# open-mmlab/Amphion

Hardware: AMD Instinct MI355X
Metric: audio samples/sec (HiFi-GAN V1 22.05 kHz generator, mel->wav) (higher is better)
Workload: dtype f32 (split-f16 MFMA: 3 x v_mfma_f32_32x32x16_f16 per term, f32 accumulate)

## Files before the change

### amphion_amd/_lib.py

```python
from __future__ import annotations

import ctypes
import os
import weakref
from ctypes import POINTER, c_char_p, c_float, c_int, c_int32, c_int64, c_size_t, c_void_p

_HERE = os.path.dirname(os.path.abspath(__file__))
LIB_PATH = os.environ.get("AMP_LIB_PATH") or os.path.join(_HERE, "lib", "libamphion_hip.so")

AMP_MAX_STAGES = 8
AMP_MAX_KERNELS = 8
AMP_MAX_DILATIONS = 8

AMP_ARCH_HIFIGAN, AMP_ARCH_BIGVGAN, AMP_ARCH_HIFIGAN_VITS = 0, 1, 2
AMP_ACT_LRELU, AMP_ACT_SNAKE, AMP_ACT_SNAKEBETA = 0, 1, 2
AMP_PRECISION_F32, AMP_PRECISION_F16X3 = 0, 1
AMP_CONV_OPT_PAD_REFLECT, AMP_CONV_OPT_TANH = 1, 2
AMP_PAD_REPLICATE, AMP_PAD_ZEROS, AMP_PAD_REFLECT = 0, 1, 2
AMP_PW_BIAS, AMP_PW_BIAS_GELU, AMP_PW_SCALE_RES = 0, 1, 2
PRECISIONS = {"f32": AMP_PRECISION_F32, "fp32": AMP_PRECISION_F32, "f16x3": AMP_PRECISION_F16X3}


class AmpError(RuntimeError):

# ... 19 lines not shown
        ("snake_logscale", c_int32),
        ("gin_channels", c_int32),
    ]


class amp_mel_desc(ctypes.Structure):
    _fields_ = [
        ("struct_size", ctypes.c_uint32),
        ("n_fft", c_int32),
        ("win_size", c_int32),
        ("hop_size", c_int32),
        ("n_mel", c_int32),
        ("pad_mode", c_int32),
        ("mag_eps", c_float),
        ("log_clip", c_float),
        ("mel_bands_dev", c_void_p),
        ("range_dev", c_void_p),
        ("range_host", c_void_p),
        ("range_reset_dev", c_void_p),
        ("range_seq", c_int32),
    ]

    def __init__(self, *args, **kw):
        super().__init__(ctypes.sizeof(type(self)), *args, **kw)


class amp_dw_desc(ctypes.Structure):
    _fields_ = [
        ("residual_channels", c_int32),
        ("residual_layers", c_int32),
        ("dilation_cycle_length", c_int32),
        ("n_mel", c_int32),
        ("upsample0", c_int32),
        ("upsample1", c_int32),
        ("max_steps", c_int32),
    ]


_SIGNATURES = {
    "amp_version": (c_int, []),
    "amp_last_error": (c_char_p, []),
    "amp_device_count": (c_int, []),
    "amp_set_precision": (c_int, [c_int]),
    "amp_get_precision": (c_int, []),
    "amp_gen_create": (c_int, [POINTER(amp_gen_desc), POINTER(c_void_p)]),
    "amp_gen_set_weight": (c_int, [c_void_p, c_char_p, c_void_p, POINTER(c_int64), c_int]),
    "amp_gen_finalize": (c_int, [c_void_p]),
    "amp_gen_hop": (c_int, [c_void_p]),
    "amp_gen_workspace_bytes": (c_size_t, [c_void_p, c_int, c_int]),
    "amp_set_group_mb": (c_int, [c_int]),
    "amp_set_pair_strips": (c_int, [c_int]),
    "amp_set_strip_fit": (c_int, [c_int]),
    "amp_pair_strip_plan": (c_int, [c_int, c_int, c_int, c_int, POINTER(c_int), POINTER(c_int), POINTER(c_int), POINTER(c_int)]),
    "amp_range_check": (c_int, [c_void_p]),
    "amp_gen_range_check": (c_int, [c_void_p, c_void_p]),
    "amp_gen_forward": (c_int, [c_void_p, c_void_p, c_void_p, c_int, c_int, c_void_p, c_void_p, c_size_t, c_void_p]),
    "amp_gen_forward_ragged": (c_int, [c_void_p, c_void_p, c_void_p, c_void_p, c_int, c_int, c_void_p, c_void_p, c_size_t, c_void_p]),
    "amp_gen_set_profiling": (c_int, [c_void_p, c_int]),
    "amp_gen_last_timing_ms": (c_int, [c_void_p, c_int, POINTER(c_float)]),
    "amp_gen_timing_ms": (c_int, [c_void_p, c_int, c_int, POINTER(c_float)]),
    "amp_gen_kernel_name": (c_int, [c_void_p, c_int, c_int, c_char_p, c_size_t]),
    "amp_gen_destroy": (None, [c_void_p]),
    "amp_conv_create": (c_int, [c_int, c_int, c_int, c_int, c_int, c_int, c_int, c_void_p, c_void_p, POINTER(c_void_p)]),
    "amp_conv_out_len": (c_int, [c_void_p, c_int]),
    "amp_conv_forward": (c_int, [c_void_p, c_void_p, c_int, c_int, c_float, c_void_p, c_float, c_void_p, c_void_p]),
    "amp_conv_forward_strided": (c_int, [c_void_p, c_void_p, ctypes.c_longlong, c_int, c_int, c_float, c_void_p, c_float, c_void_p, c_void_p]),
    "amp_conv_forward_ragged": (c_int, [c_void_p, c_void_p, ctypes.c_longlong, c_int, c_int, c_void_p, c_float, c_void_p, c_float, c_void_p, c_void_p]),
    "amp_conv_forward_mrf": (c_int, [c_void_p, c_void_p, c_int, c_int, c_float, c_void_p, c_void_p, c_int, c_float, c_void_p]),
    "amp_apnet_polar": (c_int, [c_void_p, c_void_p, c_void_p, c_size_t, c_void_p, c_void_p, c_void_p, c_void_p]),
    "amp_istft_same": (c_int, [POINTER(amp_mel_desc), c_void_p, c_void_p, c_int, c_int, c_void_p, c_void_p, c_void_p, c_void_p, c_void_p]),
    "amp_istft_same_polar": (c_int, [POINTER(amp_mel_desc), c_void_p, ctypes.c_longlong, c_int, c_int, c_float, c_void_p, c_void_p, c_void_p,
                                     c_void_p, c_void_p]),
    "amp_pw_create": (c_int, [c_int, c_int, c_void_p, c_void_p, POINTER(c_void_p)]),
    "amp_pw_forward": (c_int, [c_void_p, c_void_p, ctypes.c_longlong, c_int, c_int, c_int, c_void_p, c_void_p, c_void_p, c_void_p]),
    "amp_pw_precision": (c_int, [c_void_p]),
    "amp_pw_destroy": (None, [c_void_p]),
    "amp_dw_create": (c_int, [POINTER(amp_dw_desc), POINTER(c_void_p)]),
    "amp_dw_set_weight": (c_int, [c_void_p, c_char_p, c_void_p, ctypes.c_longlong]),
    "amp_dw_finalize": (c_int, [c_void_p]),
    "amp_dw_precision": (c_int, [c_void_p]),
    "amp_dw_set_precision": (c_int, [c_void_p, c_int]),
    "amp_dw_workspace_bytes": (c_size_t, [c_void_p, c_int, c_int]),
    "amp_dw_condition": (c_int, [c_void_p, c_void_p, c_int, c_int, c_void_p, c_void_p, c_size_t, c_void_p]),
    "amp_dw_embed": (c_int, [c_void_p, c_void_p, c_int, c_void_p, c_void_p]),
    "amp_dw_input": (c_int, [c_void_p, c_void_p, c_int, c_int, c_void_p, c_void_p]),
    "amp_dw_layer": (c_int, [c_void_p, c_int, c_void_p, c_void_p, c_void_p, ctypes.c_longlong, c_void_p, c_void_p, c_void_p, c_int, c_int, c_void_p]),
    "amp_dw_tail": (c_int, [c_void_p, c_void_p, c_int, c_int, c_void_p, c_void_p]),
    "amp_dw_forward": (c_int, [c_void_p, c_void_p, c_int, c_void_p, c_int, c_void_p, c_int, c_int, c_void_p, c_void_p, c_size_t, c_void_p]),
    "amp_dw_sample_step": (c_int, [c_void_p, c_void_p, c_int, c_float, c_float, c_float, c_float, c_void_p, c_void_p, c_int, c_int, c_void_p,
                                   c_size_t, c_void_p]),
    "amp_dw_destroy": (None, [c_void_p]),
    "amp_fvq_create": (c_int, [c_int, c_int, c_int, c_int, c_int, POINTER(c_void_p), POINTER(c_void_p), POINTER(c_void_p), POINTER(c_void_p),
                               POINTER(c_void_p), POINTER(c_void_p)]),
    "amp_fvq_encode": (c_int, [c_void_p, c_void_p, c_int, c_int, c_int, c_void_p, c_void_p, c_void_p, c_void_p]),
    "amp_fvq_decode": (c_int, [c_void_p, c_void_p, c_int, c_int, c_int, c_void_p, c_void_p]),
    "amp_fvq_check": (c_int, [c_void_p, c_void_p]),
    "amp_fvq_encode_ex": (c_int, [c_void_p, c_void_p, ctypes.c_longlong, c_void_p, c_int, c_int, c_int, c_void_p, c_void_p, c_void_p, c_void_p,
                                  c_void_p]),
    "amp_fvq_decode_add": (c_int, [c_void_p, c_void_p, c_int, c_int, c_int, c_void_p, c_void_p, c_void_p]),
    "amp_semantic_prepare": (c_int, [c_void_p, c_void_p, c_void_p, c_int, c_int, c_int, c_int, c_void_p, c_void_p]),
    "amp_fvq_destroy": (None, [c_void_p]),
    "amp_codec_unit_create": (c_int, [c_int, c_int, c_void_p, c_void_p, c_void_p, c_void_p, c_void_p, c_void_p, POINTER(c_void_p)]),
    "amp_codec_unit_fused": (c_int, [c_void_p]),
    "amp_set_codec_unit_fusion": (c_int, [c_int]),
    "amp_codec_unit_workspace_bytes": (c_size_t, [c_void_p, c_int, c_int]),
    "amp_codec_unit_forward": (c_int, [c_void_p, c_void_p, c_int, c_int, c_void_p, c_void_p, c_size_t, c_void_p]),
# ... 248 lines not shown
```

### amphion_amd/csrc/amp_host.h

```cpp
#pragma once
#include <math.h>

#include <vector>

#include "amp_internal.h"

#define AMP_HIP(expr)                                                                  \
    do {                                                                               \
        hipError_t e__ = (expr);                                                       \
        if (e__ != hipSuccess) {                                                       \
            set_error("%s failed: %s (%s:%d)", #expr, hipGetErrorString(e__), __FILE__, __LINE__); \
            return AMP_ERR_HIP;                                                        \
        }                                                                              \
    } while (0)

#define AMP_RC(expr) do { int rc__ = (expr); if (rc__ != AMP_OK) return rc__; } while (0)

struct amp_conv {
    int transposed = 0, cin = 0, cout = 0, k = 0, stride = 1, dilation = 1, padding = 0;
    int M = 0, ntaps = 0, KT = 0, off0 = 0, dstep = 0, halo_left = 0, halo_right = 0, up = 1, up_pad = 0;
    int nchunks = 0;
    int precision = amp::PREC_F32;
    int pad_reflect = 0, tanh_out = 0;
    int out_pad = 0;
// ... 4 lines not shown
    void* wp_dev = nullptr;
    float* bias_dev = nullptr;
    ~amp_conv() {
        if (wp_dev) (void)hipFree(wp_dev);
        if (bias_dev) (void)hipFree(bias_dev);
    }
};

struct amp_pw {
    int cin = 0, cout = 0;
    int precision = amp::PREC_F16X3;
    int nsteps = 0;
    float inv_scale = 1.f;
    uint4* wp_dev = nullptr;
    float* bias_dev = nullptr;
    amp_conv* conv = nullptr;
    ~amp_pw() {
        if (wp_dev) (void)hipFree(wp_dev);
        if (bias_dev) (void)hipFree(bias_dev);
        delete conv;
    }
};

namespace amp {

int device_upload(const void* host, size_t bytes, void** out);

struct DeviceAllocs {
    std::vector<void*> owned;
    DeviceAllocs() = default;
    DeviceAllocs(const DeviceAllocs&) = delete;
    DeviceAllocs& operator=(const DeviceAllocs&) = delete;
    ~DeviceAllocs() {
        for (void* p : owned) (void)hipFree(p);
    }
    int upload(const void* host, size_t bytes, void** out) {
        if (int rc = device_upload(host, bytes, out); rc != AMP_OK) return rc;
        owned.push_back(*out);
        return AMP_OK;
    }
    template <class T, class P>
    int upload(const std::vector<T>& v, P** out) { return upload(v.data(), v.size() * sizeof(T), (void**)out); }
};

int default_precision();

constexpr int kConvBlkDefault = 3;
constexpr int kConvRgFastDefault = 1;
constexpr int kPingPongDefault = 1;
struct Config {
    int pair_strips = -1;
    int strip_fit = -1;
    int rb_fusion = 1;
    int ampb_fusion = 1;
    int conv_blk = kConvBlkDefault;
    size_t group_bytes = 0;
    int small_conv = 1;
    int conv_rg_fast = 1;
    int pingpong = 1;
    int narrow_blk = 1;
    int rb_streams = -1;
    Config();
};
Config& cfg();

struct RangeGuard {
    unsigned* dev = nullptr;
    unsigned* host = nullptr;
    hipEvent_t ev = nullptr;
    bool pending = false;
};
bool guard_init(RangeGuard& g);
void guard_free(RangeGuard& g);
int range_poll(RangeGuard* g, hipStream_t st);
int range_publish(RangeGuard* g, hipStream_t st);
int range_check_sync(RangeGuard* g, hipStream_t st, const char* who);
struct RangeFlagScope {
    explicit RangeFlagScope(unsigned* word);
    ~RangeFlagScope();
    RangeFlagScope(const RangeFlagScope&) = delete;
    RangeFlagScope& operator=(const RangeFlagScope&) = delete;
};

inline float pow2_weight_scale(float wmax) {
    int e2 = 0;
    if (wmax > 0.f) { (void)frexpf(wmax, &e2); if (ldexpf(1.f, e2 - 1) == wmax) e2 -= 1; }
    return wmax > 0.f ? ldexpf(1.f, 13 - e2) : 1.f;
}

template <class View>
std::vector<_Float16> pack_a_f16x3(int row_blocks, int k16, int taps, size_t pad_entries, float wscale, View view) {
    std::vector<_Float16> wp(((size_t)row_blocks * k16 * taps * 2 + pad_entries) * 64 * 8, (_Float16)0.f);
    for (int mb = 0; mb < row_blocks; ++mb)
        for (int c = 0; c < k16; ++c)
            for (int g = 0; g < taps; ++g)
                for (int lane = 0; lane < 64; ++lane)
                    for (int e = 0; e < 8; ++e) {
                        const float v = view(mb * 32 + (lane & 31), c * 16 + 8 * (lane >> 5) + e, g) * wscale;
                        const _Float16 hi = (_Float16)v;
                        const _Float16 lo = (_Float16)(v - (float)hi);
                        const size_t ent = (((size_t)mb * k16 + c) * taps + g) * 2;
                        wp[((ent + 0) * 64 + lane) * 8 + e] = hi;
                        wp[((ent + 1) * 64 + lane) * 8 + e] = lo;
                    }
    return wp;
}

template <class View>
int pack_matrix_f16x3(const char* who, int rows, int cols, int row_blocks, int k16, View W, std::vector<_Float16>* wp, float* inv_scale) {
    float wmax = 0.f;
    for (int m = 0; m < rows; ++m)
        for (int i = 0; i < cols; ++i) {
            const float w = fabsf(W(m, i));
            if (!(w < 1e30f)) { set_error("%s: non-finite weight", who); return AMP_ERR_INVALID; }
            wmax = fmaxf(wmax, w);
        }
    const float wscale = pow2_weight_scale(wmax);
    *inv_scale = 1.f / (16.f * wscale);
    *wp = pack_a_f16x3(row_blocks, k16, 1, 0, wscale, [&](int m, int i, int) { return (m < rows && i < cols) ? W(m, i) : 0.f; });
    return AMP_OK;
}

int conv_build(amp_conv* c, const float* w, const float* bias);
int conv_run(const amp_conv* c, const float* x, int B, int T, float slope_in, const float* res, float slope_out, float* y, int mode, float div,
             hipStream_t stream, long long xbs = 0, const int* lens = nullptr, int len_mul = 1, ConvArgs* plan_small = nullptr,
             int* plan_ni = nullptr);
int next_rev(const int* lens);

bool pair_supported(const amp_conv* c1, const amp_conv* c2);
int pair_run(const amp_conv* c1, const amp_conv* c2, const float* x, int B, int T, float slope, float* y, int mode, float div,
             hipStream_t stream, const int* lens = nullptr, int len_mul = 1);
bool pair_strip_plan(int B, int T, int k, bool ragged, int* form, int* strip_len, int* spi, int* steps);
bool pair_tile_args(const amp_conv* c1, const amp_conv* c2, const float* x, int B, int T, float slope, float* y, int mode, float div,
                    const int* lens, int len_mul, PairArgs* out);

bool rb_supported(const amp_conv* const* c1, const amp_conv* const* c2, int np, int B, int T);
int rb_split(const amp_conv* const* c1, int np, int B, int T);
int rb_run(const amp_conv* const* c1, const amp_conv* const* c2, int np, const float* x, int B, int T, float slope, float* y, int mode,
           float div, hipStream_t stream, const int* lens = nullptr, int len_mul = 1, int first = 0, int count = -1);

struct ActParams {
    float* a_dev = nullptr;
    float* invb_dev = nullptr;
    float* fu_dev = nullptr;
    float* fd_dev = nullptr;
    float* fu2_dev = nullptr;
};
int act_params_upload(const float* alpha_dev, const float* beta_dev, int C, int logscale, const float* filt_up_host,
                      const float* filt_down_host, float** out);
bool ampb_supported(const amp_conv* const* c1, const amp_conv* const* c2, int np, const ActParams* acts, size_t nacts, int B, int T);
int ampb_run(const amp_conv* const* c1, const amp_conv* const* c2, int np, const ActParams* acts, const float* x, int B, int T, float* y,
             int mode, float div, hipStream_t stream, const int* lens = nullptr, int len_mul = 1);

}
```

### amphion_amd/csrc/amp_internal.h

```cpp
#pragma once
#include <hip/hip_runtime.h>
#include <stdarg.h>
#include <stdint.h>
#include <stdio.h>

#include <atomic>
#include <mutex>
#include <string>
#include <vector>

#include "amphion_hip.h"

namespace amp {

constexpr int KC = 8;
constexpr int KC16 = 16;

enum { PREC_F32 = 0, PREC_F16X3 = 1 };

struct ConvArgs {
    const float* x;
    const void* wp;
    const float* bias;
    const float* res;
// ... 27 lines not shown
    float* wn_x;
    float* wn_out;
    int wn_first, wn_last;
};

struct PairArgs {
    const float* x;
    float* y;
    const void* wp1;
    const float* bias1;
    const void* wp2;
    const float* bias2;
    int B, C, T;
    int tiles_per_item;
    int strip_len;
    int strips_per_item;
    int wide;
    int fit;
    int rev;
    int dil;
    float slope;
    float sc1, isc1, sc2, isc2;
    int mode;
    float div;
    const int* lens;
    int len_mul;
    unsigned* range_flag;
};

struct ConvSmall3Args {
    ConvArgs a[3];
    int nx[3], ny[3];
};
hipError_t launch_conv_small3(const ConvSmall3Args& p, const int ni[3], hipStream_t stream);

struct Pair3Args {
    PairArgs a[3];
    int n[3];
};
hipError_t launch_pair3(const Pair3Args& p, hipStream_t stream);

constexpr int AMP_RB_MAX_PAIRS = 3;
struct RbArgs {
    const float* x;
    float* y;
    const void* wp1[AMP_RB_MAX_PAIRS];
    const float* bias1[AMP_RB_MAX_PAIRS];
    const void* wp2[AMP_RB_MAX_PAIRS];
    const float* bias2[AMP_RB_MAX_PAIRS];
    float sc1[AMP_RB_MAX_PAIRS], isc1[AMP_RB_MAX_PAIRS], sc2[AMP_RB_MAX_PAIRS], isc2[AMP_RB_MAX_PAIRS];
    int dil[AMP_RB_MAX_PAIRS];
    int np;
    int rh;
    int B, C, T;
    int tiles_per_item;
    int rev;
    float slope;
    int mode;
    float div;
    const int* lens;
    int len_mul;
    unsigned* range_flag;
};

constexpr int AMP_AMPB_MAX_STEPS = 6;
struct AmpbArgs {
    const float* x;
    float* y;
    const void* wp[AMP_AMPB_MAX_STEPS];
    const float* bias[AMP_AMPB_MAX_STEPS];
    float sc[AMP_AMPB_MAX_STEPS], isc[AMP_AMPB_MAX_STEPS];
    int dil[AMP_AMPB_MAX_STEPS];
    const float* act_a[AMP_AMPB_MAX_STEPS];
    const float* act_invb[AMP_AMPB_MAX_STEPS];
    const float* act_fu[AMP_AMPB_MAX_STEPS];
    const float* act_fd[AMP_AMPB_MAX_STEPS];
    int ns;
    int rh;
    int B, C, T;
    int tiles_per_item;
    int rev;
    int mode;
    float div;
    const int* lens;
    int len_mul;
    unsigned* range_flag;
};

constexpr int DW_TN = 64;
struct DwLayerArgs {
    const float* x;
    const float* cond;
    const float* dconst;
    long long dconst_bs;
    const float* skip_in;
    float* x_out;
    float* skip_out;
    const uint4* wp1;
    const uint4* wp2;
    const float* w1f;
    const float* w2f;
    const float* bias1;
    const float* bias2;
    int C, n_mel, L, d;
    int K16;
    int tiles_per_item;
// ... 211 lines not shown
```

### amphion_amd/csrc/conv_host.hip

```cpp
#include <string.h>

#include <memory>
#include <type_traits>
#include <vector>

#include "amp_host.h"

namespace amp {

template <int... K> struct Taps { static constexpr int list[] = {K...}; };
using ConvTaps = Taps<1, 2, 3, 5, 7, 11>;
using BlkTaps = Taps<2, 3, 7, 11>;
using SmallTaps = Taps<1, 3, 5, 7, 11>;
using PairTaps = Taps<3, 5, 7, 11>;
using RbTaps = Taps<3, 5, 7, 11>;
using AmpbTaps = Taps<3, 5, 7, 11>;

template <int... K, typename R, typename F>
static R with_taps(Taps<K...>, int k, R dflt, F&& f) {
    R r = dflt;
    (void)((k == K && (r = f(std::integral_constant<int, K>{}), true)) || ...);
    return r;
}

// ... 376 lines not shown
    }
    const int NT = pair_tile(c1->k, c1->cin, c1->dilation);
    if (NT <= 0) return false;
    a.tiles_per_item = (T + NT - 1) / NT;
    *out = a;
    return true;
}

static int rb_fusion_mode() { return cfg().rb_fusion; }
static int rb_form(int C, int k) {
    const int m = rb_fusion_mode();
    if (m == 0) return -1;
    if (m == 3) return (C == 32 || (C == 64 && k <= 5)) ? 0 : 1;
    if (m == 2) return 1;
    if (C == 32) return k >= 11 ? 1 : 0;
    if (C == 64) return k <= 5 ? 0 : 1;
    if (C == 128) return 1;
    return -1;
}
constexpr long long kRbMinWorkgroups = 256;

bool rb_supported(const amp_conv* const* c1, const amp_conv* const* c2, int np, int B, int T) {
    if (np < 1 || np > AMP_RB_MAX_PAIRS) return false;
    int max_dil = 1, rh = 0;
    for (int p = 0; p < np; ++p) {
        if (!c1[p] || !c2[p] || !pair_supported(c1[p], c2[p])) return false;
        if (c1[p]->cin != c1[0]->cin || c1[p]->k != c1[0]->k) return false;
        max_dil = c1[p]->dilation > max_dil ? c1[p]->dilation : max_dil;
        rh += (c1[p]->k - 1) / 2 * (c1[p]->dilation + 1);
    }
    const int form = rb_form(c1[0]->cin, c1[0]->k);
    if (form < 0) return false;
    const int W = rb_tile(c1[0]->k, c1[0]->cin, max_dil, form);
    if (W <= 0 || W - 2 * rh < W / 2) return false;
    const int NT = W - 2 * rh;
    if (rb_fusion_mode() == 1 && (long long)B * ((T + NT - 1) / NT) < kRbMinWorkgroups) return false;
    return true;
}

int rb_split(const amp_conv* const* c1, int np, int B, int T) {
    if (np != 3 || rb_fusion_mode() != 1) return 0;
    int max_dil = 1, rh = 0;
    for (int p = 0; p < np; ++p) {
        max_dil = c1[p]->dilation > max_dil ? c1[p]->dilation : max_dil;
        rh += (c1[p]->k - 1) / 2 * (c1[p]->dilation + 1);
    }
    const int W = rb_tile(c1[0]->k, c1[0]->cin, max_dil, rb_form(c1[0]->cin, c1[0]->k));
    const int NT = W - 2 * rh;
    if (W <= 0 || 5 * NT >= 4 * W) return 0;
    if ((long long)B * ((T + NT - 1) / NT) < 1024) return 0;
    return 2;
}

int rb_run(const amp_conv* const* c1, const amp_conv* const* c2, int np, const float* x, int B, int T, float slope, float* y, int mode,
           float div, hipStream_t stream, const int* lens, int len_mul, int first, int count) {
    if (x == y) { set_error("rb_run: x and y must not alias"); return AMP_ERR_INVALID; }
    if (slope > 1.f) { set_error("rb_run: leaky_relu slope %g > 1 is outside the fused kernels", (double)slope); return AMP_ERR_UNSUPPORTED; }
    RbArgs a{};
    a.x = x; a.y = y;
    a.np = count < 0 ? np - first : count;
    c1 += first;
    c2 += first;
    int max_dil = 1;
    for (int p = 0; p < a.np; ++p) {
        a.wp1[p] = c1[p]->wp_dev; a.bias1[p] = c1[p]->bias_dev; a.wp2[p] = c2[p]->wp_dev; a.bias2[p] = c2[p]->bias_dev;
        a.sc1[p] = 16.f * c1[p]->wscale; a.isc1[p] = 1.f / a.sc1[p];
        a.sc2[p] = 16.f * c2[p]->wscale; a.isc2[p] = 1.f / a.sc2[p];
        a.dil[p] = c1[p]->dilation;
        a.rh += (c1[p]->k - 1) / 2 * (c1[p]->dilation + 1);
        max_dil = c1[p]->dilation > max_dil ? c1[p]->dilation : max_dil;
    }
    for (int p = a.np; p < AMP_RB_MAX_PAIRS; ++p) {
        a.wp1[p] = a.wp1[0]; a.bias1[p] = a.bias1[0]; a.wp2[p] = a.wp2[0]; a.bias2[p] = a.bias2[0]; a.dil[p] = 1;
    }
    a.B = B; a.C = c1[0]->cin; a.T = T;
    const int form = rb_form(a.C, c1[0]->k);
    const int W = rb_tile(c1[0]->k, a.C, max_dil, form);
    const int NT = W - 2 * a.rh;
    a.tiles_per_item = (T + NT - 1) / NT;
    a.slope = slope; a.mode = mode; a.div = div;
    a.lens = lens; a.len_mul = len_mul;
    a.range_flag = range_flag_for_current_device();
    a.rev = next_rev(lens);
    AMP_HIP(launch_rb(c1[0]->k, a, form, stream));
    return AMP_OK;
}

static int ampb_fusion_mode() { return cfg().ampb_fusion; }
static int ampb_form(int C, int k) {
    const int m = ampb_fusion_mode();
    if (m == 0) return -1;
    if (m == 3) return C == 32 ? 0 : 1;
    if (m == 2) return 1;
    if (C == 32) return k >= 11 ? 1 : 0;
    if (C == 64) return k <= 3 ? 1 : -1;
    return -1;
}
constexpr long long kAmpbMinWorkgroups = 256;

static int ampb_halo(const amp_conv* const* c1, int np) {
    int rh = 0;
    for (int p = 0; p < np; ++p) rh += 10 + (c1[p]->k - 1) / 2 * (c1[p]->dilation + 1);
    return (rh + 3) & ~3;
}

bool ampb_supported(const amp_conv* const* c1, const amp_conv* const* c2, int np, const ActParams* acts, size_t nacts, int B, int T) {
    if (np < 1 || 2 * np > AMP_AMPB_MAX_STEPS || nacts != (size_t)(2 * np)) return false;
    for (size_t i = 0; i < nacts; ++i)
        if (!acts[i].fu2_dev) return false;
    if ((T & 3) != 0) return false;
    int max_dil = 1;
    for (int p = 0; p < np; ++p) {
        const amp_conv *a = c1[p], *b = c2[p];
        if (!a || !b || a->precision != PREC_F16X3 || b->precision != PREC_F16X3) return false;
        if (a->pad_reflect || b->pad_reflect || a->tanh_out || b->tanh_out || a->transposed || b->transposed) return false;
        if (a->cin != a->cout || b->cin != b->cout || a->cin != b->cin || a->cin != c1[0]->cin) return false;
        if (a->k != c1[0]->k || b->k != a->k || b->dilation != 1 || a->k != a->KT) return false;
        if (a->padding != (a->k - 1) / 2 * a->dilation || b->padding != (b->k - 1) / 2) return false;
        if (!a->bias_dev || !b->bias_dev) return false;
        max_dil = a->dilation > max_dil ? a->dilation : max_dil;
    }
    const int form = ampb_form(c1[0]->cin, c1[0]->k);
    if (form < 0) return false;
    const int W = ampb_tile(c1[0]->k, c1[0]->cin, max_dil, form);
    const int rh = ampb_halo(c1, np);
    if (W <= 0 || W - 2 * rh < W / 2) return false;
    const int NT = W - 2 * rh;
    if (ampb_fusion_mode() == 1 && (long long)B * ((T + NT - 1) / NT) < kAmpbMinWorkgroups) return false;
    return true;
}
// ... 261 lines not shown
```

### amphion_amd/csrc/rb_f16x3.hip

```cpp
#include "f16x3_device.h"

#ifndef AMP_KT
#error "compile with -DAMP_KT=<taps>"
#endif

namespace amp {


template <int KT, int WM, int WN, int NI, int RING = 0, int RB_G = 32>
__global__ __launch_bounds__(64 * WM * WN, 2) void rb_f16x3_kernel(const RbArgs a) {
    static_assert(RING == 0 || RING < KT, "a ring shorter than one chunk");
    constexpr int NTHR = 64 * WM * WN;
    constexpr int W = 32 * NI * WN;
    constexpr int WL = W + 2 * RB_G;
    constexpr int H2 = (KT - 1) / 2;
    constexpr int NCH = 2 * WM;
    constexpr int CHS = 4 * WL;
    constexpr int C = 32 * WM;
    static_assert(NI % 2 == 0, "B fragments are read in halves");
    extern __shared__ __attribute__((aligned(16))) uint4 smem4[];

    const int tid = threadIdx.x;
    const int lane = tid & 63;
    const int wave = __builtin_amdgcn_readfirstlane(tid >> 6);
    const int wm = wave / WN, wn = wave % WN;
    const int hi = lane >> 5, l31 = lane & 31;
    const int nbx = gridDim.x;
    int bx = tile_order(blockIdx.x, nbx, a.lens != nullptr, a.rev);
    const int item = bx / a.tiles_per_item;
    const int tile = bx - item * a.tiles_per_item;
    const int T = a.T;
    const int RH = a.rh;
    const int NT = W - 2 * RH;
    const int O0 = tile * NT;
    int Tv = T;
    if (a.lens) { const int l = a.lens[item] * a.len_mul; Tv = l < Tv ? l : Tv; }
    if (O0 >= Tv) return;
    const int q0 = O0 - RH;

    for (int i = tid; i < NCH * 4 * 2 * RB_G; i += NTHR) {
        const int row = i / (2 * RB_G), g = i - row * (2 * RB_G);
        smem4[row * WL + (g < RB_G ? g : W + g)] = make_uint4(0u, 0u, 0u, 0u);
    }

    const int colw = wn * (32 * NI) + l31;
    int qcl[NI];
    bool qok[NI];
#pragma unroll
    for (int t = 0; t < NI; ++t) {
        const int q = q0 + colw + 32 * t;
        qok[t] = (q >= 0) && (q < Tv);
        qcl[t] = q < 0 ? 0 : (q < T ? q : T - 1);
    }
    const float* xr = a.x + (size_t)item * C * T + (size_t)(32 * wm + 16 * hi) * T;
    f32x16 rv[NI];
#pragma unroll
    for (int t = 0; t < NI; ++t)
#pragma unroll
        for (int r = 0; r < 16; ++r) rv[t][r] = xr[(size_t)r * T + qcl[t]];

    constexpr size_t MBS = (size_t)NCH * (KT * 128);
    constexpr int NA = RING > 0 ? RING : KT;
    Frag a_h[NA], a_l[NA];
    const int wlane = (lane & 32) | (16 * ((lane >> 2) & 1) + 4 * ((lane >> 3) & 3) + (lane & 3));
    {
        const uint4* w0 = static_cast<const uint4*>(a.wp1[0]) + (size_t)wm * MBS + wlane;
#pragma unroll
        for (int g = 0; g < NA; ++g) {
            a_h[g].u = w0[g * 128];
            a_l[g].u = w0[g * 128 + 64];
        }
    }
    AMP_PIN_VMEM();

    float range_max = 0.f;
    const float kpos = 16.f, kneg = 16.f * a.slope;
    auto stage_x = [&]() __attribute__((always_inline)) {
#pragma unroll
        for (int t = 0; t < NI; ++t) {
            const int col = RB_G + colw + 32 * t;
            const bool ok = qok[t];
            const int o4 = (2 * wm + hi) * CHS + col;
#pragma unroll
            for (int o = 0; o < 2; ++o) {
                struct { uint2 u; } fh0, fl0, fh1, fl1;
                stage4_f16(ok ? rv[t][8 * o + 0] : 0.f, ok ? rv[t][8 * o + 1] : 0.f, ok ? rv[t][8 * o + 2] : 0.f,
                           ok ? rv[t][8 * o + 3] : 0.f, kpos, kneg, range_max, fh0.u, fl0.u);
                stage4_f16(ok ? rv[t][8 * o + 4] : 0.f, ok ? rv[t][8 * o + 5] : 0.f, ok ? rv[t][8 * o + 6] : 0.f,
                           ok ? rv[t][8 * o + 7] : 0.f, kpos, kneg, range_max, fh1.u, fl1.u);
                smem4[o4 + o * WL] = make_uint4(fh0.u.x, fh0.u.y, fh1.u.x, fh1.u.y);
                smem4[o4 + o * WL + 2 * WL] = make_uint4(fl0.u.x, fl0.u.y, fl1.u.x, fl1.u.y);
            }
        }
    };

    f32x16 acc[NI];
    auto conv = [&](const void* wp, const float* bias, float sc, int d, const void* wp_next) __attribute__((always_inline)) {
#pragma unroll
        for (int r = 0; r < 16; ++r) {
            const float bv = bias[32 * wm + 16 * hi + r] * sc;
#pragma unroll
            for (int t = 0; t < NI; ++t) acc[t][r] = bv;
        }
        const uint4* wa = static_cast<const uint4*>(wp) + (size_t)wm * MBS + wlane;
        const uint4* wn0 = static_cast<const uint4*>(wp_next) + (size_t)wm * MBS + wlane;
        const int rd = hi * WL + RB_G + colw - H2 * d;
#pragma unroll 1
        for (int c = 0; c < NCH; ++c) {
            const uint4* wcur = wa + (size_t)c * (KT * 128);
            const uint4* wan = (c + 1) < NCH ? wa + (size_t)(c + 1) * (KT * 128) : wn0;
            const uint4* base = smem4 + c * CHS + rd;
#pragma unroll
            for (int g = 0; g < KT; ++g) {
                const int v = RING > 0 ? g % NA : g;
                const uint4* bg = base + g * d;
                constexpr int NB = NI / 2;
#pragma unroll
                for (int th = 0; th < 2; ++th) {
                    Frag bh[NB], bl[NB];
#pragma unroll
                    for (int t = 0; t < NB; ++t) {
                        bh[t].u = bg[32 * (th * NB + t)];
                        bl[t].u = bg[2 * WL + 32 * (th * NB + t)];
                    }
                    mfma3<NB>(acc + th * NB, a_h[v], a_l[v], bh, bl);
                }
                {
                    const bool same = RING > 0 && g + RING < KT;
                    const uint4* src = same ? wcur + (size_t)(g + RING) * 128 : wan + (size_t)v * 128;
                    a_h[v].u = src[0];
                    a_l[v].u = src[64];
                }
                AMP_PIN_VMEM();
            }
        }
    };

    stage_x();
    __syncthreads();

    const int np = a.np;
#pragma unroll 1
    for (int p = 0; p < AMP_RB_MAX_PAIRS; ++p) {
        if (p < np) {
            const bool last = (p + 1 == np);
            conv(a.wp1[p], a.bias1[p], a.sc1[p], a.dil[p], a.wp2[p]);
            __syncthreads();
            {
                const float i1 = a.isc1[p];
                const float slope = a.slope;
#pragma unroll
                for (int t = 0; t < NI; ++t) {
                    const int o4 = (2 * wm + hi) * CHS + RB_G + colw + 32 * t;
#pragma unroll
                    for (int o = 0; o < 2; ++o) {
                        struct { uint2 u; } fh0, fl0, fh1, fl1;
                        seam4_f16(acc[t][8 * o + 0], acc[t][8 * o + 1], acc[t][8 * o + 2], acc[t][8 * o + 3], i1, slope, qok[t], range_max, fh0.u, fl0.u);
                        seam4_f16(acc[t][8 * o + 4], acc[t][8 * o + 5], acc[t][8 * o + 6], acc[t][8 * o + 7], i1, slope, qok[t], range_max, fh1.u, fl1.u);
                        smem4[o4 + o * WL] = make_uint4(fh0.u.x, fh0.u.y, fh1.u.x, fh1.u.y);
                        smem4[o4 + o * WL + 2 * WL] = make_uint4(fl0.u.x, fl0.u.y, fl1.u.x, fl1.u.y);
                    }
                }
            }
            __syncthreads();
            conv(a.wp2[p], a.bias2[p], a.sc2[p], 1, last ? a.wp2[p] : a.wp1[p + 1 < AMP_RB_MAX_PAIRS ? p + 1 : p]);
            {
                const float i2 = a.isc2[p];
#pragma unroll
                for (int t = 0; t < NI; ++t)
#pragma unroll
                    for (int r = 0; r < 16; ++r) rv[t][r] = __builtin_fmaf(acc[t][r], i2, rv[t][r]);
            }
            if (!last) {
                __syncthreads();
                stage_x();
                __syncthreads();
            }
        }
    }

    {
        const int mode = a.mode;
        float* yr = a.y + (size_t)item * C * T + (size_t)(32 * wm + 16 * hi) * T;
        if (mode != 0) {
#pragma unroll
            for (int t = 0; t < NI; ++t)
#pragma unroll
                for (int r = 0; r < 16; ++r) acc[t][r] = yr[(size_t)r * T + qcl[t]];
#pragma unroll
            for (int t = 0; t < NI; ++t) rv[t] += acc[t];
            if (mode == 2) {
#pragma unroll
                for (int t = 0; t < NI; ++t)
#pragma unroll
                    for (int r = 0; r < 16; ++r) rv[t][r] = rv[t][r] / a.div;
            }
        }
#pragma unroll
        for (int t = 0; t < NI; ++t) {
            const int col = colw + 32 * t;
// ... 53 lines not shown
```

### amphion_amd/csrc/runtime.hip

```cpp
#include <stdarg.h>
#include <stdio.h>
#include <stdlib.h>
#include <string.h>

#include <mutex>
#include <string>

#include "amp_host.h"

namespace amp {

static thread_local char g_err[512] = "";

void set_error(const char* fmt, ...) {
    va_list ap;
    va_start(ap, fmt);
    vsnprintf(g_err, sizeof(g_err), fmt, ap);
    va_end(ap);
}

static RangeGuard g_guard[64];
__thread std::string* tl_kernel_log = nullptr;
__thread char tl_last_kernel[160] = "";
__thread int tl_conv_transposed = 0;
// ... 64 lines not shown

int range_poll(RangeGuard* g, hipStream_t st) {
    if (!g || !g->dev || !g->pending || stream_is_capturing(st)) return AMP_OK;
    if (hipEventQuery(g->ev) != hipSuccess) return AMP_OK;
    g->pending = false;
    if (*g->host == 0) return AMP_OK;
    *g->host = 0;
    AMP_HIP(hipMemsetAsync(g->dev, 0, sizeof(unsigned), st));
    set_error("%s", kRangeMsg);
    return AMP_ERR_RANGE;
}

int range_publish(RangeGuard* g, hipStream_t st) {
    if (!g || !g->dev || stream_is_capturing(st)) return AMP_OK;
    AMP_HIP(hipMemcpyAsync(g->host, g->dev, sizeof(unsigned), hipMemcpyDeviceToHost, st));
    AMP_HIP(hipEventRecord(g->ev, st));
    g->pending = true;
    return AMP_OK;
}

int range_check_sync(RangeGuard* g, hipStream_t st, const char* who) {
    if (!g || !g->dev) return AMP_OK;
    if (stream_is_capturing(st)) { set_error("%s: the stream is capturing", who); return AMP_ERR_STATE; }
    AMP_HIP(hipMemcpyAsync(g->host, g->dev, sizeof(unsigned), hipMemcpyDeviceToHost, st));
    AMP_HIP(hipStreamSynchronize(st));
    g->pending = false;
    const unsigned v = *g->host;
    *g->host = 0;
    if (v == 0) return AMP_OK;
    AMP_HIP(hipMemsetAsync(g->dev, 0, sizeof(unsigned), st));
    set_error("%s", kRangeMsg);
    return AMP_ERR_RANGE;
}

static int g_precision = -1;
int default_precision() {
    if (g_precision < 0) {
        const char* e = getenv("AMP_PRECISION");
        g_precision = (e && (!strcmp(e, "f32") || !strcmp(e, "fp32"))) ? PREC_F32 : PREC_F16X3;
    }
    return g_precision;
}

Config::Config() {
    auto num = [](const char* name, int lo, int hi, int dflt) {
        const char* e = getenv(name);
        if (!e || !*e) return dflt;
        const int v = atoi(e);
        return (v < lo || v > hi) ? dflt : v;
    };
    rb_fusion = num("AMP_RB_FUSION", 0, 3, 1);
    ampb_fusion = num("AMP_AMPB_FUSION", 0, 3, 1);
    rb_streams = num("AMP_RB_STREAMS", -1, 1, -1);
    static const char* const kRemoved[][2] = {
        {"AMP_GROUP_MB", "amp_set_group_mb(megabytes)"}, {"AMP_PAIR_STRIP", "amp_set_pair_strips(mode)"}, {"AMP_CONV_BLK", "amp_set_conv_blk(mode)"},
        {"AMP_FUSE_PAIRS", "nothing (the fused pairs are the only form)"}, {"AMP_RB_SUM_FRAMES", "nothing"},
        {"AMP_RB_HORIZONTAL", "amp_set_resblock_streams(mode)"}, {"AMP_RB_HORIZONTAL_FRAMES", "amp_set_resblock_streams(mode)"}};
    for (const auto& r : kRemoved) {
        const char* e = getenv(r[0]);
        if (e && *e) fprintf(stderr, "libamphion_hip: the environment variable %s=%s is no longer read (removed in ABI 142); use %s\n", r[0], e, r[1]);
    }
}
Config& cfg() { static Config c; return c; }

int device_upload(const void* host, size_t bytes, void** out) {
    void* p = nullptr;
    AMP_HIP(hipMalloc(&p, bytes));
    const hipError_t e = hipMemcpy(p, host, bytes, hipMemcpyHostToDevice);
    if (e != hipSuccess) {
        (void)hipFree(p);
        set_error("hipMemcpy of %zu bytes to the device failed: %s", bytes, hipGetErrorString(e));
        return AMP_ERR_HIP;
    }
    *out = p;
    return AMP_OK;
}

}

using namespace amp;

extern "C" {

int amp_version(void) { return 158; }
const char* amp_last_error(void) { return g_err; }

int amp_set_precision(int precision) {
    if (precision != AMP_PRECISION_F32 && precision != AMP_PRECISION_F16X3) {
        set_error("amp_set_precision: unknown precision %d", precision);
        return AMP_ERR_INVALID;
    }
    g_precision = precision;
    return AMP_OK;
}

int amp_get_precision(void) { return default_precision(); }

int amp_device_count(void) {
    int n = 0;
    if (hipGetDeviceCount(&n) != hipSuccess) return 0;
    return n;
}

int amp_set_pair_strips(int on) {
    if (on < -1 || on > 0) { set_error("amp_set_pair_strips: %d (-1 the policy, 0 the per-tile kernel everywhere; the four-wave strips of mode 1 left in ABI 142)", on); return AMP_ERR_INVALID; }
    cfg().pair_strips = on;
    return AMP_OK;
}

int amp_set_strip_fit(int mode) {
    if (mode < -1 || mode > 1) { set_error("amp_set_strip_fit: %d (-1 the plan, 0 never: shifted strips, 1 every strip launch)", mode); return AMP_ERR_INVALID; }
    cfg().strip_fit = mode;
    return AMP_OK;
}

int amp_pair_strip_plan(int B, int T, int k, int ragged, int* form, int* strip_len, int* strips_per_item, int* steps) {
    if (B < 1 || T < 1 || !form || !strip_len || !strips_per_item || !steps) { set_error("amp_pair_strip_plan: B=%d T=%d or a null result pointer", B, T); return AMP_ERR_INVALID; }
    if (!pair_strip_plan(B, T, k, ragged != 0, form, strip_len, strips_per_item, steps)) { set_error("amp_pair_strip_plan: no strip kernel for k=%d", k); return AMP_ERR_UNSUPPORTED; }
    return AMP_OK;
}

int amp_set_group_mb(int megabytes) {
    if (megabytes < 0) { set_error("amp_set_group_mb: %d", megabytes); return AMP_ERR_INVALID; }
    cfg().group_bytes = (size_t)megabytes << 20;
    return AMP_OK;
}

int amp_set_resblock_streams(int mode) {
    if (mode < -1 || mode > 1) { set_error("amp_set_resblock_streams: mode=%d", mode); return AMP_ERR_INVALID; }
    cfg().rb_streams = mode;
    return AMP_OK;
}

int amp_set_small_conv(int on) {
    cfg().small_conv = on ? 1 : 0;
    return AMP_OK;
}

int amp_set_pingpong(int on) {
    cfg().pingpong = on < 0 ? kPingPongDefault : (on ? 1 : 0);
    return AMP_OK;
}

int amp_set_conv_rg_fast(int on) {
    cfg().conv_rg_fast = on < 0 ? kConvRgFastDefault : (on ? 1 : 0);
    return AMP_OK;
}

int amp_set_conv_blk_narrow(int on) {
    if (on < -1 || on > 2) { set_error("amp_set_conv_blk_narrow: %d (0 off, 1 policy: 128-row convs with k >= 7, 2 every 128-row conv, -1 default)", on); return AMP_ERR_INVALID; }
    cfg().narrow_blk = on < 0 ? 1 : on;
    return AMP_OK;
}

int amp_set_conv_blk(int mode) {
    if (mode < -1 || mode > 3) { set_error("amp_set_conv_blk: mode %d (0 off, 1 | 2 chunks per staging round, 3 = 2 + k = 7 / 11, -1 default)", mode); return AMP_ERR_INVALID; }
    cfg().conv_blk = mode < 0 ? kConvBlkDefault : mode;
    return AMP_OK;
}

int amp_set_resblock_fusion(int mode) {
    if (mode < -1 || mode > 3) { set_error("amp_set_resblock_fusion: mode=%d", mode); return AMP_ERR_INVALID; }
    cfg().rb_fusion = mode < 0 ? 1 : mode;
    return AMP_OK;
}

int amp_set_ampblock_fusion(int mode) {
    if (mode < -1 || mode > 3) { set_error("amp_set_ampblock_fusion: mode=%d", mode); return AMP_ERR_INVALID; }
    cfg().ampb_fusion = mode < 0 ? 1 : mode;
    return AMP_OK;
}

int amp_range_check(void* stream_) {
    return range_check_sync(guard_for_current_device(), (hipStream_t)stream_, "amp_range_check");
// ... 4 lines not shown
```

### include/amphion_hip.h

```cpp
#ifndef AMPHION_HIP_H
#define AMPHION_HIP_H

#include <stddef.h>
#include <stdint.h>

#ifdef __cplusplus
extern "C" {
#endif

typedef enum amp_status {
    AMP_OK = 0,
    AMP_ERR_INVALID = -1,
    AMP_ERR_MISSING_WEIGHT = -2,
    AMP_ERR_HIP = -3,
    AMP_ERR_UNSUPPORTED = -4,
    AMP_ERR_STATE = -5,
    AMP_ERR_RANGE = -6
} amp_status;

typedef enum amp_arch {
    AMP_ARCH_HIFIGAN = 0,
    AMP_ARCH_BIGVGAN = 1,
    AMP_ARCH_HIFIGAN_VITS = 2
} amp_arch;
// ... 109 lines not shown
int amp_dwconv_layer_norm_c_causal(const float* x_dev, const float* dw_weight_dev, const float* dw_bias_dev, int K, int dilation,
                                   const float* gamma_dev, const float* beta_dev, const int* lens_dev, int B, int C, int T, float eps,
                                   int gelu, float* y_dev, void* stream);
int amp_dds_seam(const float* y_dev, const float* x_dev, const float* gamma2_dev, const float* beta2_dev, float eps2,
                 const float* dw_weight_dev, const float* dw_bias_dev, int K, int dilation, const float* gamma1_dev, const float* beta1_dev,
                 float eps1, const int* lens_dev, int B, int C, int T, float* x_out_dev, float* z_out_dev, void* stream);
int amp_add_channel_bias(float* x_dev, const float* cb_dev, int B, int C, int T, void* stream);
int amp_rel_attention(const float* q_dev, const float* k_dev, const float* v_dev, const float* emb_k_dev,
                      const float* emb_v_dev, const int* lens_dev, int B, int H, int dk, int T, int window, float* out_dev,
                      void* stream);
int amp_rel_attention_strided(const float* q_dev, const float* k_dev, const float* v_dev, long long qkv_batch_stride,
                              const float* emb_k_dev, const float* emb_v_dev, const int* lens_dev, int B, int H, int dk, int T,
                              int window, float* out_dev, void* stream);
int amp_set_rel_attention_tiled(int on);
int amp_dwconv(const float* x_dev, const float* w_dev, const float* bias_dev, const int* lens_dev, int B, int C, int T, int K,
               int dilation, float* y_dev, void* stream);
int amp_spline_flow(const float* z_dev, const float* h_dev, const int* lens_dev, int B, int T, int num_bins,
                    int filter_channels, float tail_bound, int inverse, int flip_in, int flip_out, float* z_out_dev,
                    void* stream);
int amp_spline_flow_proj(const float* z_dev, const float* hc_dev, const float* proj_w_dev, const float* proj_b_dev, const int* lens_dev,
                         int B, int C, int T, int num_bins, int filter_channels, float tail_bound, int inverse, int flip_in, int flip_out,
                         float* z_out_dev, void* stream);
int amp_affine_reverse(const float* x_dev, const float* m_dev, const float* logs_dev, const int* lens_dev, int B, int C, int T,
                       float* y_dev, void* stream);
int amp_embed_tokens(const long long* tokens_dev, const float* weight_dev, const int* lens_dev, int B, int T, int hidden,
                     int n_vocab, float scale, float* y_dev, void* stream);
int amp_embed_sum_c(const long long* codes_dev, int N, const float* const* tables, const int* rows, int D, const float* init_dev, int B, int T,
                    float* y_dev, unsigned* flag_dev, void* stream);
int amp_embed_sum_check(unsigned* flag_dev, void* stream);
int amp_durations(const float* logw_dev, const int* lens_dev, int B, int T, float length_scale, float* w_ceil_dev, int* cum_dev,
                  int* ylen_dev, void* stream);
int amp_expand_path(const float* src_dev, const int* cum_dev, const int* xlens_dev, const int* ylens_dev, int B, int D, int Tx,
                    int Ty, float* out_dev, float* attn_dev, void* stream);
int amp_expand_path_strided(const float* src_dev, long long src_batch_stride, const int* cum_dev, const int* xlens_dev,
                            const int* ylens_dev, int B, int D, int Tx, int Ty, float* out_dev, float* attn_dev, void* stream);
int amp_gauss_sample(const float* m_dev, const float* logs_dev, const float* noise_dev, size_t n, float noise_scale,
                     float* out_dev, void* stream);

int amp_snake(const float* x_dev, int B, int C, int T, const float* alpha_dev, const float* beta_dev, int logscale,
              float* y_dev, void* stream);

int amp_wav_to_pcm16(const float* wav_dev, int B, int L, long long wav_stride, const int* lens_dev, int16_t* pcm_dev,
                     long long pcm_stride, void* stream);

typedef enum amp_conv_option { AMP_CONV_OPT_PAD_REFLECT = 1, AMP_CONV_OPT_TANH = 2 } amp_conv_option;
int amp_conv_set_option(amp_conv* c, int option, int value);

int amp_pair_forward(const amp_conv* c1, const amp_conv* c2, const float* x_dev, int B, int T, float slope,
                     float* y_dev, void* stream);

int amp_resblock_forward(const amp_conv* const* c1, const amp_conv* const* c2, int n_pairs, const float* x_dev, int B, int T,
                         float slope, float* y_dev, void* stream);
int amp_set_resblock_fusion(int mode);
int amp_set_resblock_streams(int mode);
int amp_gen_prepare_streams(amp_gen* g);

int amp_ampblock_forward(const amp_conv* const* c1, const amp_conv* const* c2, int n_pairs, const float* alpha_dev,
                         const float* beta_dev, int logscale, const float* filt_up_host, const float* filt_down_host,
                         const float* x_dev, int B, int T, float* y_dev, int mode, float div, void* stream);
int amp_set_ampblock_fusion(int mode);

void amp_conv_destroy(amp_conv* c);

int amp_set_small_conv(int on);

int amp_set_conv_blk(int mode);
int amp_set_conv_blk_narrow(int on);

int amp_set_conv_rg_fast(int on);

int amp_set_pingpong(int on);


int amp_conv_create_gated(int hidden, int k, int dilation, int padding, const float* weight_host, const float* bias_host,
                          amp_conv** out);

int amp_wn_forward(const amp_conv* const* in_layers, const amp_conv* const* res_skip_layers, int n_layers, float* x_dev,
                   const float* cond_dev, long long cond_batch_stride, const int32_t* lens_dev, int B, int T,
                   float* acts_ws_dev, float* out_dev, void* stream);


int amp_wn_gate(const float* a_dev, const float* cond_dev, long long cond_batch_stride, float* out_dev, int B, int H,
                int T, void* stream);
int amp_wn_accumulate(float* x_dev, float* out_dev, const float* rs_dev, const int32_t* lens_dev, int B, int H, int T,
                      int first, int last, void* stream);
int amp_sequence_mask(float* x_dev, const int32_t* lens_dev, int B, int C, int T, void* stream);
int amp_coupling_apply(float* x_dev, const float* m_dev, const int32_t* lens_dev, int B, int half_channels, int T,
                       int reverse, void* stream);
int amp_flip_channels(const float* x_dev, float* y_dev, int B, int C, int T, void* stream);
int amp_posterior_sample(const float* stats_dev, const float* eps_dev, const int32_t* lens_dev, float* z_dev, int B,
                         int C, int T, void* stream);

int amp_antialias_snake(const float* x_dev, int B, int C, int T, const float* alpha_dev, const float* beta_dev,
                        int logscale, const float* filt_up_host, const float* filt_down_host, float* y_dev,
                        void* stream);

typedef struct amp_mel_desc {
    uint32_t struct_size;
    int32_t n_fft;
    int32_t win_size;
    int32_t hop_size;
    int32_t n_mel;
    int32_t pad_mode;
    float mag_eps;
    float log_clip;
    const int32_t* mel_bands_dev;
// ... 233 lines not shown
```

Baseline: 151.2 million.

## Load real neighbour columns into ResBlock guard slots to shrink the first-pair halo

In the fused whole-ResBlock kernel, the guard columns in shared memory are now filled with real input samples (activated and split to f16) instead of zeros, for k>=7 kernels whose first dilation fits the guard width. This lets the first conv read beyond the tile edge, so the recompute halo rh drops by the first pair's reach and each tile yields more output columns, meaning fewer tiles and less redundant recompute. After the first conv the guards are re-zeroed. Each block pays a few extra strided global loads, and the change adds a plan query API and an env/setter switch.

```diff
diff --git a/amphion_amd/_lib.py b/amphion_amd/_lib.py
--- a/amphion_amd/_lib.py
+++ b/amphion_amd/_lib.py
@@ -95,6 +95,8 @@
     "amp_set_pair_strips": (c_int, [c_int]),
     "amp_set_strip_fit": (c_int, [c_int]),
     "amp_pair_strip_plan": (c_int, [c_int, c_int, c_int, c_int, POINTER(c_int), POINTER(c_int), POINTER(c_int), POINTER(c_int)]),
+    "amp_set_rb_guard": (c_int, [c_int]),
+    "amp_rb_plan": (c_int, [c_int, c_int, POINTER(c_int), c_int, c_int, c_int, c_int, c_int, POINTER(c_int), POINTER(c_int), POINTER(c_int), POINTER(c_int)]),
     "amp_range_check": (c_int, [c_void_p]),
     "amp_gen_range_check": (c_int, [c_void_p, c_void_p]),
     "amp_gen_forward": (c_int, [c_void_p, c_void_p, c_void_p, c_int, c_int, c_void_p, c_void_p, c_size_t, c_void_p]),
diff --git a/amphion_amd/csrc/amp_host.h b/amphion_amd/csrc/amp_host.h
--- a/amphion_amd/csrc/amp_host.h
+++ b/amphion_amd/csrc/amp_host.h
@@ -80,6 +80,7 @@
     int pair_strips = -1;
     int strip_fit = -1;
     int rb_fusion = 1;
+    int rb_guard = -1;
     int ampb_fusion = 1;
     int conv_blk = kConvBlkDefault;
     size_t group_bytes = 0;
@@ -164,6 +165,7 @@
 
 bool rb_supported(const amp_conv* const* c1, const amp_conv* const* c2, int np, int B, int T);
 int rb_split(const amp_conv* const* c1, int np, int B, int T);
+bool rb_plan(int C, int k, const int* dil, int n, int first, int count, int B, int T, int* form, int* W, int* rh, int* tiles_per_item);
 int rb_run(const amp_conv* const* c1, const amp_conv* const* c2, int np, const float* x, int B, int T, float slope, float* y, int mode,
            float div, hipStream_t stream, const int* lens = nullptr, int len_mul = 1, int first = 0, int count = -1);
 
diff --git a/amphion_amd/csrc/amp_internal.h b/amphion_amd/csrc/amp_internal.h
--- a/amphion_amd/csrc/amp_internal.h
+++ b/amphion_amd/csrc/amp_internal.h
@@ -103,6 +103,7 @@
     int dil[AMP_RB_MAX_PAIRS];
     int np;
     int rh;
+    int guard_x;
     int B, C, T;
     int tiles_per_item;
     int rev;
diff --git a/amphion_amd/csrc/conv_host.hip b/amphion_amd/csrc/conv_host.hip
--- a/amphion_amd/csrc/conv_host.hip
+++ b/amphion_amd/csrc/conv_host.hip
@@ -452,6 +452,36 @@
     return 2;
 }
 
+static int rb_guard_columns(int C, int form) { return ((C == 64 && form == 0) || C == 128) ? 16 : 32; }
+static void rb_geometry(int C, int k, const int* dil, int n, int form, int* rh, int* guard_x) {
+    int full = 0;
+    for (int p = 0; p < n; ++p) full += (k - 1) / 2 * (dil[p] + 1);
+    const int reach0 = (k - 1) / 2 * dil[0];
+    const int mode = cfg().rb_guard;
+    *guard_x = ((mode == 1 || (mode < 0 && k >= 7)) && reach0 <= rb_guard_columns(C, form)) ? 1 : 0;
+    *rh = *guard_x ? full - reach0 : full;
+}
+
+bool rb_plan(int C, int k, const int* dil, int n, int first, int count, int B, int T, int* form, int* W, int* rh, int* tiles_per_item) {
+    if (count < 0) count = n - first;
+    if (n < 1 || n > AMP_RB_MAX_PAIRS || first < 0 || count < 1 || first + count > n || B < 1 || T < 1) return false;
+    int max_dil = 1;
+    for (int p = 0; p < count; ++p) {
+        if (dil[first + p] < 1) return false;
+        max_dil = dil[first + p] > max_dil ? dil[first + p] : max_dil;
+    }
+    *form = rb_form(C, k);
+    if (*form < 0) return false;
+    *W = rb_tile(k, C, max_dil, *form);
+    if (*W <= 0) return false;
+    int guard_x = 0;
+    rb_geometry(C, k, dil + first, count, *form, rh, &guard_x);
+    const int NT = *W - 2 * *rh;
+    if (NT <= 0) return false;
+    *tiles_per_item = (T + NT - 1) / NT;
+    return true;
+}
+
 int rb_run(const amp_conv* const* c1, const amp_conv* const* c2, int np, const float* x, int B, int T, float slope, float* y, int mode,
            float div, hipStream_t stream, const int* lens, int len_mul, int first, int count) {
     if (x == y) { set_error("rb_run: x and y must not alias"); return AMP_ERR_INVALID; }
@@ -467,7 +497,6 @@
         a.sc1[p] = 16.f * c1[p]->wscale; a.isc1[p] = 1.f / a.sc1[p];
         a.sc2[p] = 16.f * c2[p]->wscale; a.isc2[p] = 1.f / a.sc2[p];
         a.dil[p] = c1[p]->dilation;
-        a.rh += (c1[p]->k - 1) / 2 * (c1[p]->dilation + 1);
         max_dil = c1[p]->dilation > max_dil ? c1[p]->dilation : max_dil;
     }
     for (int p = a.np; p < AMP_RB_MAX_PAIRS; ++p) {
@@ -476,6 +505,7 @@
     a.B = B; a.C = c1[0]->cin; a.T = T;
     const int form = rb_form(a.C, c1[0]->k);
     const int W = rb_tile(c1[0]->k, a.C, max_dil, form);
+    rb_geometry(a.C, c1[0]->k, a.dil, a.np, form, &a.rh, &a.guard_x);
     const int NT = W - 2 * a.rh;
     a.tiles_per_item = (T + NT - 1) / NT;
     a.slope = slope; a.mode = mode; a.div = div;
diff --git a/amphion_amd/csrc/rb_f16x3.hip b/amphion_amd/csrc/rb_f16x3.hip
--- a/amphion_amd/csrc/rb_f16x3.hip
+++ b/amphion_amd/csrc/rb_f16x3.hip
@@ -38,9 +38,39 @@
     if (O0 >= Tv) return;
     const int q0 = O0 - RH;
 
-    for (int i = tid; i < NCH * 4 * 2 * RB_G; i += NTHR) {
+    float range_max = 0.f;
+    const float kpos = 16.f, kneg = 16.f * a.slope;
+    constexpr int NG = NCH * 2 * 2 * RB_G;
+    static_assert(NG <= NTHR, "one guard item per thread");
+    auto guard_unit = [&](int i) __attribute__((always_inline)) {
         const int row = i / (2 * RB_G), g = i - row * (2 * RB_G);
-        smem4[row * WL + (g < RB_G ? g : W + g)] = make_uint4(0u, 0u, 0u, 0u);
+        return (row >> 1) * CHS + (row & 1) * WL + (g < RB_G ? g : W + g);
+    };
+    if (a.guard_x) {
+        if (tid < NG) {
+            const int row = tid / (2 * RB_G), g = tid - row * (2 * RB_G);
+            const int q = q0 + (g < RB_G ? g - RB_G : W + g - RB_G);
+            const bool ok = (q >= 0) && (q < Tv);
+            const float* xg = a.x + (size_t)item * C * T + (size_t)(8 * row) * T + (q < 0 ? 0 : (q < T ? q : T - 1));
+            float v[8];
+#pragma unroll
+            for (int e = 0; e < 8; ++e) v[e] = xg[(size_t)e * T];
+#pragma unroll
+            for (int e = 0; e < 8; ++e) {
+                AMP_OPAQUE(v[e]);
+                v[e] = ok ? v[e] : 0.f;
+            }
+            struct { uint2 u; } fh0, fl0, fh1, fl1;
+            stage4_f16(v[0], v[1], v[2], v[3], kpos, kneg, range_max, fh0.u, fl0.u);
+            stage4_f16(v[4], v[5], v[6], v[7], kpos, kneg, range_max, fh1.u, fl1.u);
+            const int o4 = guard_unit(tid);
+            smem4[o4] = make_uint4(fh0.u.x, fh0.u.y, fh1.u.x, fh1.u.y);
+            smem4[o4 + 2 * WL] = make_uint4(fl0.u.x, fl0.u.y, fl1.u.x, fl1.u.y);
+        }
+    } else if (tid < NG) {
+        const int o4 = guard_unit(tid);
+        smem4[o4] = make_uint4(0u, 0u, 0u, 0u);
+        smem4[o4 + 2 * WL] = make_uint4(0u, 0u, 0u, 0u);
     }
 
     const int colw = wn * (32 * NI) + l31;
@@ -73,8 +103,6 @@
     }
     AMP_PIN_VMEM();
 
-    float range_max = 0.f;
-    const float kpos = 16.f, kneg = 16.f * a.slope;
     auto stage_x = [&]() __attribute__((always_inline)) {
 #pragma unroll
         for (int t = 0; t < NI; ++t) {
@@ -146,6 +174,15 @@
             const bool last = (p + 1 == np);
             conv(a.wp1[p], a.bias1[p], a.sc1[p], a.dil[p], a.wp2[p]);
             __syncthreads();
+            if (p == 0 && a.guard_x) {
+                int i = tid;
+                asm volatile("" : "+v"(i));
+                if (i < NG) {
+                    const int o4 = guard_unit(i);
+                    smem4[o4] = make_uint4(0u, 0u, 0u, 0u);
+                    smem4[o4 + 2 * WL] = make_uint4(0u, 0u, 0u, 0u);
+                }
+            }
             {
                 const float i1 = a.isc1[p];
                 const float slope = a.slope;
diff --git a/amphion_amd/csrc/runtime.hip b/amphion_amd/csrc/runtime.hip
--- a/amphion_amd/csrc/runtime.hip
+++ b/amphion_amd/csrc/runtime.hip
@@ -140,6 +140,7 @@
     rb_fusion = num("AMP_RB_FUSION", 0, 3, 1);
     ampb_fusion = num("AMP_AMPB_FUSION", 0, 3, 1);
     rb_streams = num("AMP_RB_STREAMS", -1, 1, -1);
+    rb_guard = num("AMP_RB_GUARD", -1, 1, -1);
     static const char* const kRemoved[][2] = {
         {"AMP_GROUP_MB", "amp_set_group_mb(megabytes)"}, {"AMP_PAIR_STRIP", "amp_set_pair_strips(mode)"}, {"AMP_CONV_BLK", "amp_set_conv_blk(mode)"},
         {"AMP_FUSE_PAIRS", "nothing (the fused pairs are the only form)"}, {"AMP_RB_SUM_FRAMES", "nothing"},
@@ -170,7 +171,7 @@
 
 extern "C" {
 
-int amp_version(void) { return 158; }
+int amp_version(void) { return 159; }
 const char* amp_last_error(void) { return g_err; }
 
 int amp_set_precision(int precision) {
@@ -208,6 +209,21 @@
     return AMP_OK;
 }
 
+int amp_set_rb_guard(int mode) {
+    if (mode < -1 || mode > 1) { set_error("amp_set_rb_guard: %d (-1 the plan, 0 never: zero guards, 1 every whole-ResBlock launch)", mode); return AMP_ERR_INVALID; }
+    cfg().rb_guard = mode;
+    return AMP_OK;
+}
+
+int amp_rb_plan(int C, int k, const int* dilations, int n, int first, int count, int B, int T, int* form, int* tile_w, int* rh, int* tiles_per_item) {
+    if (!dilations || !form || !tile_w || !rh || !tiles_per_item) { set_error("amp_rb_plan: a null pointer"); return AMP_ERR_INVALID; }
+    if (!rb_plan(C, k, dilations, n, first, count, B, T, form, tile_w, rh, tiles_per_item)) {
+        set_error("amp_rb_plan: no whole-ResBlock launch for C=%d k=%d pairs [%d, %d) of %d, B=%d T=%d under the current switches", C, k, first, first + count, n, B, T);
+        return AMP_ERR_UNSUPPORTED;
+    }
+    return AMP_OK;
+}
+
 int amp_set_group_mb(int megabytes) {
     if (megabytes < 0) { set_error("amp_set_group_mb: %d", megabytes); return AMP_ERR_INVALID; }
     cfg().group_bytes = (size_t)megabytes << 20;
diff --git a/include/amphion_hip.h b/include/amphion_hip.h
--- a/include/amphion_hip.h
+++ b/include/amphion_hip.h
@@ -185,6 +185,9 @@
 int amp_resblock_forward(const amp_conv* const* c1, const amp_conv* const* c2, int n_pairs, const float* x_dev, int B, int T,
                          float slope, float* y_dev, void* stream);
 int amp_set_resblock_fusion(int mode);
+int amp_set_rb_guard(int mode);
+int amp_rb_plan(int C, int k, const int* dilations, int n, int first, int count, int B, int T, int* form, int* tile_w, int* rh,
+                int* tiles_per_item);
 int amp_set_resblock_streams(int mode);
 int amp_gen_prepare_streams(amp_gen* g);
 
```

Result: no change. 152.4 million (median of 6 runs) (+0.8%).
